# JoergBitzer/JadeSpectrogram

Measured on AMD Instinct MI355X. Metric: STFT frames/sec (1024-pt, 50% hop), higher is better.
Workload: dtype f32

## Files before the change

### include/jsg.h

```cpp
#ifndef JSG_H_
#define JSG_H_

#include <stddef.h>
#include <stdint.h>

#if defined(__GNUC__)
#define JSG_API __attribute__((visibility("default")))
#else
#define JSG_API
#endif

#ifdef __cplusplus
extern "C" {
#endif

#define JSG_ABI_VERSION 6

typedef enum jsg_status {
    JSG_OK = 0,
    JSG_ERR_SIZE_MISMATCH = -1,
    JSG_ERR_INVALID = -2,
    JSG_ERR_UNSUPPORTED = -3,
    JSG_ERR_HIP = -4,
    JSG_ERR_NO_DEVICE = -5,
// ... 34 lines not shown
JSG_API int jsg_plan_create(jsg_plan** out, int n, const float* window, float power_scale);
JSG_API int jsg_plan_destroy(jsg_plan* plan);
JSG_API int jsg_plan_fft_size(const jsg_plan* plan);

typedef struct jsg_stft_args {
    const float* in;
    int64_t in_pitch;
    int32_t channels;
    int32_t hop;
    int32_t feedblocks;
    int32_t mix_mode;
    int64_t first_frame;
    int64_t n_frames;
    float* out_db;
    int64_t out_pitch;
    int64_t out_channel_pitch;
    int32_t ring_width;
    int32_t ring_pos;
    int32_t linear_out;
    int32_t blocks_per_cu;
    int64_t in_samples;
    int32_t plan_select;
    int32_t exact_log;
    int32_t reserved0;
    float* out_tail;
} jsg_stft_args;
JSG_API int jsg_stft_db_launch(const jsg_plan* plan, const jsg_stft_args* args, void* stream);
JSG_API int jsg_stft_kernel_name(const jsg_plan* plan, const jsg_stft_args* args, char* out, int out_len);

JSG_API int jsg_stft_db_launch_many(const jsg_plan* plan, const jsg_stft_args* args, int count, void* const* streams, int n_streams);
JSG_API int jsg_stft_db_launch_many_threads(const jsg_plan* plan, const jsg_stft_args* args, int count, void* const* streams,
                                    int n_streams, int n_threads);

JSG_API int jsg_stft_db_launch_batches(const jsg_plan* plan, const jsg_stft_args* args, int count, void* stream);

JSG_API int jsg_stft_db_launch_strided(const jsg_plan* plan, const jsg_stft_args* args, int n_batches, int64_t in_batch_stride,
                               int64_t out_batch_stride, void* stream);
JSG_API int jsg_stft_db_strided_kernel_name(const jsg_plan* plan, const jsg_stft_args* args, int n_batches, int64_t in_batch_stride, char* out,
                                    int out_len);

JSG_API int jsg_db_from_power_launch(const float* power, float* out, int64_t count, float divisor, void* stream);
JSG_API int jsg_db_from_power_launch_ex(const float* power, float* out, int64_t count, float divisor, int exact_log, void* stream);

JSG_API int jsg_columns_from_tail_layout_launch(const float* db, int64_t db_pitch, const float* tail, int n_columns, int height, float* dst,
                                        int64_t dst_pitch, void* stream);

JSG_API int jsg_calib_copy_launch(const void* src, void* dst, int64_t bytes, void* stream);

typedef struct jsg_colormap_args {
    const float* db;
    int64_t db_pitch;
    int32_t ring_width;
    int32_t height;
    int32_t col_first;
    int32_t n_cols;
    int32_t x_first;
    int32_t x_wrap;
    const int32_t* lut;
    int32_t n_colors;
    float vmin, vmax, access_mult;
    uint32_t* argb_out;
    int64_t argb_pitch;
// ... 186 lines not shown
```

### jadespectrogram_amd/__init__.py

```python
from . import capi
from .capi import JsgError
from .spectrogram import (CColorPalette, Filterbank, FreqAxis, Plan, Spectrogram, SpectrogramDisplay, StftLaunch, colormap, colormap_lut,
                          colormap_axis, colormap_range, columns_from_tail_layout, feed_samples, memsize_blocks, next_power_of_2, stft_db, stft_db_batches, stft_db_strided, stft_db_strided_kernel_name, stft_image, stft_image_needs_scratch, stft_image_strided, stft_image_strided_needs_scratch, stft_kernel_name, window,
                          mel_spectrogram_db, stft_fb_db, stft_fb_db_strided, stft_fb_kernel_name, stft_fb_scratch_floats,
                          CStftPlan, cstft, istft, istft_launch, istft_nola, istft_scratch_floats, stft,
                          phase_vocoder, phase_vocoder_launch, pvoc_frames, time_stretch)

__all__ = ["Spectrogram", "SpectrogramDisplay", "CColorPalette", "Plan", "stft_db", "colormap", "window", "colormap_lut",
           "colormap_range", "feed_samples", "memsize_blocks", "next_power_of_2", "JsgError", "capi",
           "Filterbank", "stft_fb_db", "stft_fb_db_strided", "stft_fb_kernel_name", "mel_spectrogram_db", "FreqAxis", "colormap_axis",
           "CStftPlan", "cstft", "istft_launch", "istft_nola", "istft_scratch_floats", "stft", "istft",
           "pvoc_frames", "phase_vocoder_launch", "phase_vocoder", "time_stretch"]
```

### jadespectrogram_amd/_build.py

```python
from __future__ import annotations

import os
import shutil
import subprocess
import sys

PKG = os.path.dirname(os.path.abspath(__file__))
ROOT = os.path.dirname(PKG)
CSRC = os.path.join(PKG, "csrc")
LIB = os.path.join(PKG, "libjsg.so")

SOURCES = ["jsg_kernels.hip", "jsg_stft_a.hip", "jsg_stft_b.hip", "jsg_filterbank.hip", "jsg_display_axis.hip", "jsg_cstft.hip", "jsg_pvoc.hip", "jsg_engine.cpp", "jsg_host_math.cpp", "jsg_filterbank_host.cpp",
           "jsg_display_axis_host.cpp"]
HEADERS = ["jsg_internal.h", "jsg_block_queue.h", "jsg_exact_math.h", "jsg_stft_kernel.h", "jsg_colormap_tables.inc", os.path.join(ROOT, "include", "jsg.h")]
HIP_FLAGS = ["-fno-slp-vectorize", "-mllvm", "-amdgpu-kernarg-preload-count=16"]
VISIBILITY = ["-fvisibility=hidden", "-fvisibility-inlines-hidden"]
UNIT_FLAGS = {"jsg_stft_a.hip": ["-mllvm", "-amdgpu-sched-strategy=max-ilp"]}
ARCH = "gfx950"


def _hipcc() -> str:
    for cand in (os.environ.get("HIPCC"), shutil.which("hipcc"), "/opt/rocm/bin/hipcc"):
        if cand and os.path.exists(cand):
            return cand
    raise RuntimeError("hipcc not found: libjsg.so cannot be built (there is no CPU fallback)")


def _stale(target: str, deps) -> bool:
    if not os.path.exists(target):
        return True
    t = os.path.getmtime(target)
    return any(os.path.getmtime(d) > t for d in deps)


def build_variant(name: str, hip_flags, verbose: bool = False) -> str:
    hipcc = _hipcc()
    vdir = os.path.join(ROOT, "tools", "variants")
# ... 81 lines not shown
```

### jadespectrogram_amd/capi.py

```python
from __future__ import annotations

import ctypes as C
import os

PKG = os.path.dirname(os.path.abspath(__file__))
LIB_PATH = os.path.join(PKG, "libjsg.so")

JSG_OK = 0
JSG_ERR_SIZE_MISMATCH = -1
JSG_ERR_INVALID = -2
JSG_ERR_UNSUPPORTED = -3
JSG_ERR_HIP = -4
JSG_ERR_NO_DEVICE = -5
JSG_ERR_NOMEM = -6

MIX_ABSMEAN, MIX_MAX, MIX_MIN, MIX_LEFT, MIX_RIGHT = range(5)
MIX_PER_CHANNEL = 100
MIX_SUM = 101
WIN_RECT, WIN_HANN, WIN_HAMMING, WIN_BLACKMANHARRIS, WIN_FLATTOP, WIN_HANNPOISSON = range(6)
FEED_100, FEED_50, FEED_25, FEED_10 = range(4)
CM_MONO, CM_BW, CM_HOT, CM_RAINBOW, CM_VIRIDIS, CM_PLASMA, CM_JADE = range(7)
FB_MEL_SLANEY, FB_MEL_HTK, FB_LOG, FB_LINEAR = range(4)
FB_NORM_NONE, FB_NORM_SLANEY, FB_NORM_UNIT_SUM = range(3)
FB_MAX_BANDS = 8192
AXIS_BINS, AXIS_LINEAR, AXIS_LOG, AXIS_MEL = range(4)
AXIS_MAX_HEIGHT = 16384


class JsgError(RuntimeError):
    def __init__(self, code: int, msg: str):
        super().__init__(f"jsg error {code}: {msg}")
        self.code = code


class StftArgs(C.Structure):
    _fields_ = [("in_", C.c_void_p), ("in_pitch", C.c_int64), ("channels", C.c_int32), ("hop", C.c_int32),
                ("feedblocks", C.c_int32), ("mix_mode", C.c_int32), ("first_frame", C.c_int64),
                ("n_frames", C.c_int64), ("out_db", C.c_void_p), ("out_pitch", C.c_int64),
                ("out_channel_pitch", C.c_int64), ("ring_width", C.c_int32), ("ring_pos", C.c_int32),
                ("linear_out", C.c_int32), ("blocks_per_cu", C.c_int32), ("in_samples", C.c_int64),
                ("plan_select", C.c_int32), ("exact_log", C.c_int32), ("reserved0", C.c_int32), ("out_tail", C.c_void_p)]


class FbSpec(C.Structure):
    _fields_ = [("n", C.c_int32), ("fs", C.c_float), ("n_bands", C.c_int32), ("fmin", C.c_float), ("fmax", C.c_float),
                ("scale", C.c_int32), ("norm", C.c_int32)]


class AxisSpec(C.Structure):
    _fields_ = [("n", C.c_int32), ("fs", C.c_float), ("scale", C.c_int32), ("height", C.c_int32), ("fmin", C.c_float),
                ("fmax", C.c_float)]


class ColormapArgs(C.Structure):
    _fields_ = [("db", C.c_void_p), ("db_pitch", C.c_int64), ("ring_width", C.c_int32), ("height", C.c_int32),
                ("col_first", C.c_int32), ("n_cols", C.c_int32), ("x_first", C.c_int32), ("x_wrap", C.c_int32),
                ("lut", C.c_void_p), ("n_colors", C.c_int32), ("vmin", C.c_float), ("vmax", C.c_float),
                ("access_mult", C.c_float), ("argb_out", C.c_void_p), ("argb_pitch", C.c_int64),
                ("index_out", C.c_void_p), ("index_pitch", C.c_int64)]


class CstftArgs(C.Structure):
    _fields_ = [("in_", C.c_void_p), ("in_pitch", C.c_int64), ("rows", C.c_int32), ("hop", C.c_int32), ("n_frames", C.c_int64),
                ("in_samples", C.c_int64), ("out", C.c_void_p), ("out_frame_pitch", C.c_int64), ("out_row_pitch", C.c_int64)]
# ... 14 lines not shown
    _fields_ = [("stft", StftArgs), ("colour", ColormapArgs), ("index_scratch", C.c_void_p), ("index_scratch_pitch", C.c_int64)]


_P = C.c_void_p
SIGNATURES = {
    "jsg_abi_version": (C.c_int, []),
    "jsg_device_count": (C.c_int, []),
    "jsg_feed_samples": (C.c_int, [C.c_float, C.c_int]),
    "jsg_memsize_blocks": (C.c_int, [C.c_float, C.c_float, C.c_int]),
    "jsg_next_power_of_2": (C.c_int, [C.c_float, C.c_float]),
    "jsg_window_build": (C.c_int, [C.c_int, C.c_int, _P]),
    "jsg_colormap_build": (C.c_int, [C.c_int, C.c_int, _P]),
    "jsg_colormap_range": (C.c_int, [C.c_int, C.c_float, C.c_float, _P, _P, _P]),
    "jsg_plan_create": (C.c_int, [C.POINTER(_P), C.c_int, _P, C.c_float]),
    "jsg_plan_destroy": (C.c_int, [_P]),
    "jsg_plan_fft_size": (C.c_int, [_P]),
    "jsg_stft_db_launch": (C.c_int, [_P, C.POINTER(StftArgs), _P]),
    "jsg_stft_db_launch_many": (C.c_int, [_P, C.POINTER(StftArgs), C.c_int, C.POINTER(_P), C.c_int]),
    "jsg_stft_db_launch_many_threads": (C.c_int, [_P, C.POINTER(StftArgs), C.c_int, C.POINTER(_P), C.c_int, C.c_int]),
    "jsg_stft_db_launch_batches": (C.c_int, [_P, C.POINTER(StftArgs), C.c_int, _P]),
    "jsg_stft_kernel_name": (C.c_int, [_P, C.POINTER(StftArgs), C.c_char_p, C.c_int]),
    "jsg_stft_db_launch_strided": (C.c_int, [_P, C.POINTER(StftArgs), C.c_int, C.c_int64, C.c_int64, _P]),
    "jsg_stft_db_strided_kernel_name": (C.c_int, [_P, C.POINTER(StftArgs), C.c_int, C.c_int64, C.c_char_p, C.c_int]),
    "jsg_calib_copy_launch": (C.c_int, [_P, _P, C.c_int64, _P]),
    "jsg_columns_from_tail_layout_launch": (C.c_int, [_P, C.c_int64, _P, C.c_int, C.c_int, _P, C.c_int64, _P]),
    "jsg_colormap_launch": (C.c_int, [C.POINTER(ColormapArgs), _P]),
    "jsg_stft_image_launch": (C.c_int, [_P, C.POINTER(StftImageArgs), _P]),
    "jsg_stft_image_needs_scratch": (C.c_int, [_P, C.POINTER(StftImageArgs)]),
    "jsg_stft_image_launch_strided": (C.c_int, [_P, C.POINTER(StftImageArgs), C.c_int, C.c_int64, C.c_int64, _P]),
    "jsg_stft_image_strided_needs_scratch": (C.c_int, [_P, C.POINTER(StftImageArgs), C.c_int]),
    "jsg_db_from_power_launch": (C.c_int, [_P, _P, C.c_int64, C.c_float, _P]),
    "jsg_db_from_power_launch_ex": (C.c_int, [_P, _P, C.c_int64, C.c_float, C.c_int, _P]),
    "jsg_filterbank_build": (C.c_int, [C.POINTER(FbSpec), _P, _P, _P, _P, _P, C.c_int64, C.POINTER(C.c_int64)]),
    "jsg_filterbank_create": (C.c_int, [C.POINTER(_P), C.POINTER(FbSpec)]),
    "jsg_filterbank_create_matrix": (C.c_int, [C.POINTER(_P), C.c_int, C.c_int, _P]),
    "jsg_filterbank_destroy": (C.c_int, [_P]),
    "jsg_filterbank_bands": (C.c_int, [_P]),
    "jsg_filterbank_fft_size": (C.c_int, [_P]),
    "jsg_filterbank_weights": (C.c_int, [_P, _P]),
    "jsg_stft_fb_launch": (C.c_int, [_P, _P, C.POINTER(StftArgs), _P, C.c_int64, _P]),
    "jsg_stft_fb_launch_strided": (C.c_int, [_P, _P, C.POINTER(StftArgs), C.c_int, C.c_int64, C.c_int64, _P, C.c_int64, _P]),
    "jsg_stft_fb_scratch_floats": (C.c_int64, [_P, _P, C.POINTER(StftArgs), C.c_int]),
    "jsg_stft_fb_kernel_name": (C.c_int, [_P, _P, C.POINTER(StftArgs), C.c_int, C.c_char_p, C.c_int]),
    "jsg_freq_axis_build": (C.c_int, [C.POINTER(AxisSpec), _P, _P, _P, _P]),
    "jsg_freq_axis_create": (C.c_int, [C.POINTER(_P), C.POINTER(AxisSpec)]),
    "jsg_freq_axis_destroy": (C.c_int, [_P]),
# ... 95 lines not shown
```

### jadespectrogram_amd/csrc/jsg_kernels.hip

```cpp
#include <memory>

#include "jsg_stft_kernel.h"

namespace jsg {

#ifdef JSG_DEV_KNOBS
static int dev_knob_int(const char* name) { const char* e = getenv(name); return e ? atoi(e) : 0; }
static bool dev_knob_set(const char* name) { return getenv(name) != nullptr; }
static bool dev_knob_is(const char* name, char first) { const char* e = getenv(name); return e && e[0] == first; }
#else
static constexpr int dev_knob_int(const char*) { return 0; }
static constexpr bool dev_knob_set(const char*) { return false; }
static constexpr bool dev_knob_is(const char*, char) { return false; }
#endif

static bool chunked_traversal() {
    static const bool chunked = dev_knob_is("JSG_TRAVERSAL", 'c');
    return chunked;
}

static bool b_plan_fills_its_rounds(long long n_frames, int frames_per_workgroup, int n_cu) {
    const long long want = (n_frames + frames_per_workgroup - 1) / frames_per_workgroup;
    const long long rounds = (want + n_cu - 1) / n_cu;
    return rounds > 0 && double(want) >= kB_min_round_fill * double(rounds * n_cu);
// ... 111 lines not shown
    const long long col = blockIdx.x;
    const float* src = db + col * db_pitch;
    float* out = dst + col * dst_pitch;
    for (int k = threadIdx.x; k < half; k += 256) out[k] = src[k];
    if (threadIdx.x == 0) out[half] = tail[col];
}

__global__ __launch_bounds__(256) void calib_copy_kernel(const float* __restrict__ src, float* __restrict__ dst, long long n4) {
    typedef float v4f __attribute__((ext_vector_type(4)));
    const long long i = (long long)blockIdx.x * 256 + threadIdx.x;
    if (i < n4) __builtin_nontemporal_store(__builtin_nontemporal_load(reinterpret_cast<const v4f*>(src) + i), reinterpret_cast<v4f*>(dst) + i);
}

}

using namespace jsg;

namespace {
#define JSG_VARIANT_ROW(V, C, U, name, step, tables, pin, one_per_cu) \
    {C::N, name, step, int(Tables::tables), pin, one_per_cu, &launch_##V, &ensure_attrs_##V, &fill_tables<C>},
const VariantRow kVariants[] = {JSG_STFT_VARIANTS(JSG_VARIANT_ROW)};
#undef JSG_VARIANT_ROW
const VariantRow& row_of(Variant v) { return kVariants[int(v)]; }
}

struct jsg_plan {
    int n = 0;
    DeviceBlob blob;
    const float2* d_tab = nullptr;
    size_t set_at[kTableSets] = {0, 0, 0};
};

extern "C" {


int jsg_device_count(void) {
    int n = 0;
    if (hipGetDeviceCount(&n) != hipSuccess) return 0;
    return n;
}

static void pool_prepare_for_device(int dev);

int jsg_plan_create(jsg_plan** out, int n, const float* window, float power_scale) {
    if (!out || !window) return jsg_fail(JSG_ERR_INVALID, "jsg_plan_create: null argument");
    *out = nullptr;
// ... 40 lines not shown

int jsg_plan_fft_size(const jsg_plan* plan) { return plan ? plan->n : JSG_ERR_INVALID; }

}

int jsg::plan_device(const jsg_plan* plan) { return plan->blob.device(); }

namespace {
struct IndexOut {
    unsigned char* idx;
    long long pitch;
    float vmin, vmax, mult;
    int n_colors;
    unsigned* argb;
    long long argb_pitch;
    const int* lut;
    int x_first, x_wrap;
    int n_images = 1;
    long long in_image_stride = 0, argb_image_stride = 0;
};
}

constexpr int k1024B_min_channels = 4;

namespace {
struct CallShape {
    enum Out { kFloat, kIndex, kArgb } out = kFloat;
    long long rows = 1;
    int n_images = 1;
    bool multi_batch = false;
};
}

static Variant resolve_variant(const jsg_plan* plan, const jsg_stft_args* g, const CallShape& sh, int n_cu) {
    const int n = plan->n, mm = g->mix_mode, sel = g->plan_select;
    const bool maxmin = mm == JSG_MIX_MAX || mm == JSG_MIX_MIN;
    const int nc = (mm == JSG_MIX_LEFT || mm == JSG_MIX_RIGHT || mm == JSG_MIX_PER_CHANNEL) ? 1 : g->channels;
    if (n == 512) return Variant::k512;
    if (n == 8192) return Variant::k8192;
    if (n == 1024 && sh.out == CallShape::kArgb) return Variant::k1024I;
    if (n == 2048 && sel == 3 && sh.out == CallShape::kFloat && (mm == JSG_MIX_ABSMEAN || mm == JSG_MIX_SUM) && g->channels >= 2 &&
        (g->channels & 1) == 0)
        return Variant::k2048P;
    const Variant b_plan = n == 1024 ? Variant::k1024B : n == 2048 ? Variant::k2048B : Variant::k4096B;
    const int step = row_of(b_plan).step;
    const long long frames = sh.out == CallShape::kArgb ? (g->n_frames + step - 1) / step * step * sh.n_images : sh.rows * g->n_frames;
    bool b;
    if (n == 1024) {
        b = sh.out == CallShape::kFloat && !maxmin &&
            (sel == 2 || (sel == 0 && nc >= k1024B_min_channels && b_plan_fills_its_rounds(frames, step, n_cu)));
    } else {
        static const int forced2048 = dev_knob_int("JSG_2048_PLAN");
        static const int forced4096 = dev_knob_int("JSG_4096_PLAN");
        const int forced = sel == 1 ? 3 : sel == 2 ? 2 : n == 2048 ? forced2048 : forced4096;
        b = forced == 2 || (forced != 3 && nc >= (n == 2048 ? k2048B_min_channels : k4096B_min_channels) &&
                            b_plan_fills_its_rounds(frames, step, n_cu));
    }
    if (b) return b_plan;
    if (n == 2048) return Variant::k2048;
    if (n == 4096) return Variant::k4096;
    static const bool no_runs = dev_knob_set("JSG_NO_RUNS");
    const bool runs = sh.multi_batch && nc == 1 && !maxmin && (long long)g->hop * g->feedblocks == n && 2 * g->hop == n &&
                      !chunked_traversal() && !no_runs;
    return runs ? Variant::k1024Runs : Variant::k1024;
}

const VariantRow& jsg::strided_call_variant(const jsg_plan* plan, const jsg_stft_args* g, int n_batches, int n_cu) {
    const bool one_by_one = g->mix_mode == JSG_MIX_MAX || g->mix_mode == JSG_MIX_MIN;
    CallShape sh;
    sh.rows = (one_by_one ? 1ll : (long long)n_batches) * (g->mix_mode == JSG_MIX_PER_CHANNEL ? g->channels : 1);
    return row_of(resolve_variant(plan, g, sh, n_cu));
}

int jsg::check_stft_args(int n, const jsg_stft_args* g, const char* who) {
    if (g->hop <= 0 || g->feedblocks <= 0) return jsg_fail_who(JSG_ERR_INVALID, who, "bad geometry (hop, feedblocks)");
    if (g->channels > 65535) return jsg_fail_who(JSG_ERR_UNSUPPORTED, who, "more than 65535 channels");
    if (g->in_samples != 0) {
        const long long j = g->first_frame + g->n_frames - 1;
        const long long start = ((long long)g->hop * g->feedblocks == n) ? j * g->hop : (j / g->feedblocks) * n + (j % g->feedblocks) * g->hop;
        if (g->in_samples < 0 || start + n > g->in_samples) return jsg_fail_who(JSG_ERR_INVALID, who, "the last frame would read past the end of the input rows");
        if (g->channels > 1 && g->in_pitch < g->in_samples) return jsg_fail_who(JSG_ERR_INVALID, who, "in_pitch < in_samples");
    }
    if (g->n_frames >= (1ll << 31) || g->first_frame + g->n_frames >= (1ll << 31)) return jsg_fail_who(JSG_ERR_UNSUPPORTED, who, "frame index does not fit 31 bits");
    switch (g->mix_mode) {
        case JSG_MIX_ABSMEAN: case JSG_MIX_MAX: case JSG_MIX_MIN: case JSG_MIX_LEFT: case JSG_MIX_PER_CHANNEL: case JSG_MIX_SUM: return JSG_OK;
        case JSG_MIX_RIGHT:
            return g->channels < 2 ? jsg_fail_who(JSG_ERR_INVALID, who, "JSG_MIX_RIGHT needs at least two channels") : JSG_OK;
// ... 288 lines not shown
        one.in = g->in + b0 * in_batch_stride;
        one.out_db = g->out_db ? g->out_db + b0 * out_batch_stride : nullptr;
        if (g->out_tail) one.out_tail = g->out_tail + b0 * rows_per_batch * g->ring_width;
        if (nb == 1) rc = jsg_stft_db_launch(plan, &one, stream);
        else {
            BatchSpec bs{nb, (long long)in_batch_stride, (long long)out_batch_stride};
            rc = stft_launch_impl(plan, &one, nullptr, stream, &bs);
        }
        if (rc != JSG_OK) return rc;
    }
    return JSG_OK;
}

int jsg_stft_db_strided_kernel_name(const jsg_plan* plan, const jsg_stft_args* g, int n_batches, int64_t in_batch_stride, char* out, int out_len) {
    if (!plan || !g || !out || out_len < 24 || n_batches < 1) return jsg_fail(JSG_ERR_INVALID, "jsg_stft_db_strided_kernel_name: bad argument");
    int dev = -1;
    if (hipGetDevice(&dev) != hipSuccess) return jsg_fail(JSG_ERR_NO_DEVICE, "jsg_stft_db_strided_kernel_name: no device");
    if (n_batches == 1) return jsg_stft_kernel_name(plan, g, out, out_len);
    (void)in_batch_stride;
    std::snprintf(out, size_t(out_len), "%s", strided_call_variant(plan, g, n_batches, cu_count_of_device(dev)).name);
    return JSG_OK;
}

int jsg_stft_db_launch_many(const jsg_plan* plan, const jsg_stft_args* args, int count, void* const* streams, int n_streams) {
    if (!plan || (!args && count > 0) || count < 0 || n_streams < 0 || (n_streams > 0 && !streams))
        return jsg_fail(JSG_ERR_INVALID, "jsg_stft_db_launch_many: bad argument");
    for (int i = 0; i < count; ++i) {
        void* st = n_streams > 0 ? streams[i % n_streams] : nullptr;
        const int rc = jsg_stft_db_launch(plan, &args[i], st);
        if (rc != JSG_OK) return rc;
    }
    return JSG_OK;
}

int jsg_stft_db_launch_many_threads(const jsg_plan* plan, const jsg_stft_args* args, int count, void* const* streams, int n_streams,
                                    int n_threads) {
    if (n_threads <= 1 || n_streams <= 1) return jsg_stft_db_launch_many(plan, args, count, streams, n_streams);
    if (!plan || (!args && count > 0) || count < 0 || !streams) return jsg_fail(JSG_ERR_INVALID, "jsg_stft_db_launch_many_threads: bad argument");
    if (n_threads > n_streams) n_threads = n_streams;
    if (n_threads > 16) n_threads = 16;
    int dev = 0;
    if (hipGetDevice(&dev) != hipSuccess) return jsg_fail(JSG_ERR_NO_DEVICE, "jsg_stft_db_launch_many_threads: no device");
    std::vector<int> rcs(size_t(n_threads), JSG_OK);
    std::vector<std::string> errs{size_t(n_threads)};
    auto body = [&](int t) {
        if (hipSetDevice(dev) != hipSuccess) { rcs[size_t(t)] = JSG_ERR_HIP; return; }
// ... 193 lines not shown
```

### jadespectrogram_amd/csrc/jsg_stft_a.hip

```cpp
#include "jsg_stft_kernel.h"

namespace jsg {
#define JSG_IN_UNIT_A(...) __VA_ARGS__
#define JSG_IN_UNIT_B(...)
JSG_STFT_VARIANTS(JSG_DEFINE_VARIANT)
hipError_t touch_module_a() { return preload_code_object(reinterpret_cast<const void*>(&stft_db_kernel<Cfg1024, 3>)); }
}
```

### jadespectrogram_amd/csrc/jsg_stft_kernel.h

```cpp
#pragma once
#include <hip/hip_runtime.h>

#include <algorithm>
#include <atomic>
#include <cmath>
#include <cstdint>
#include <cstdio>
#include <cstdlib>
#include <mutex>
#include <new>
#include <string>
#include <thread>
#include <type_traits>
#include <utility>
#include <vector>

#include "../../include/jsg.h"
#include "jsg_internal.h"
#include "jsg_exact_math.h"

namespace jsg {

typedef float cf __attribute__((ext_vector_type(2)));

// ... 1499 lines not shown
    else
        hipLaunchKernelGGL((stft_db_kernel<C, MIXOP, OUTK, STREAM, 0>), grid, dim3(C::WPB * 64), lds, s, ka.in, ka.in_pitch, ka.tab, ka.n_frames,
                           ka.first_frame, ka.hop, flags, unsigned(ka.c_begin) | unsigned(ka.c_end) << 16, ka.iters, grid.x, ka.feedblocks, ka);
    return hipGetLastError();
}

template <class C, int K = 0>
hipError_t launch_stft(const StftKArgs& ka, int mixop, int stream, dim3 grid, hipStream_t s) {
    if constexpr (K == 4 * 3 * 3) return hipErrorInvalidValue;
    else {
        constexpr int MIXOP = K % 4, OUTK = K / 4 % 3, STREAM = K / 12;
        if constexpr (stft_instantiated<C, MIXOP, OUTK, STREAM>())
            if (mixop == MIXOP && (ka.argb ? 2 : ka.idx ? 1 : 0) == OUTK && stream == STREAM) return launch_stft_mix<C, MIXOP, OUTK, STREAM>(ka, grid, s);
        return launch_stft<C, K + 1>(ka, mixop, stream, grid, s);
    }
}

#define JSG_STFT_VARIANTS(X)                                                                                  \
    X(k512,      Cfg512,   A, "Cfg512",   Cfg512::TPB,            First, 0, false)                            \
    X(k1024,     Cfg1024,  A, "Cfg1024",  Cfg1024::TPB,           First, 1, false)                            \
    X(k1024I,    Cfg1024I, A, "Cfg1024I", Cfg1024I::TPB,          First, 0, false)                            \
    X(k1024B,    Cfg1024B, A, "Cfg1024B", Cfg1024B::TPB,          B,     2, true)                             \
    X(k1024Runs, Cfg1024,  A, "Cfg1024",  Cfg1024::TPB * kRunLen, First, 1, false)                            \
    X(k2048,     Cfg2048,  A, "Cfg2048",  Cfg2048::TPB,           First, 1, false)                            \
    X(k2048B,    Cfg2048B, A, "Cfg2048B", Cfg2048B::TPB,          B,     2, true)                             \
    X(k2048P,    Cfg2048P, A, "Cfg2048P", Cfg2048P::TPB,          Pair,  3, true)                             \
    X(k4096,     Cfg4096,  B, "Cfg4096",  Cfg4096::TPB,           First, 1, false)                            \
    X(k4096B,    Cfg4096B, B, "Cfg4096B", Cfg4096B::TPB,          B,     2, true)                             \
    X(k8192,     Cfg8192,  A, "Cfg8192",  Cfg8192::TPB,           First, 0, false)

#define JSG_VARIANT_ENUMERATOR(V, ...) V,
enum class Variant : int { JSG_STFT_VARIANTS(JSG_VARIANT_ENUMERATOR) };
#undef JSG_VARIANT_ENUMERATOR

#define JSG_VARIANT_ENTRY_POINTS(V, C, ...)                                                        \
    hipError_t launch_##V(const StftKArgs& ka, int mixop, bool strided, dim3 grid, hipStream_t s); \
    hipError_t ensure_attrs_##V();
JSG_STFT_VARIANTS(JSG_VARIANT_ENTRY_POINTS)
#undef JSG_VARIANT_ENTRY_POINTS
enum class Tables : int { First, B, Pair };
constexpr int kTableSets = 3;
struct VariantRow {
    int n;
    const char* name;
    int step;
    int tables;
    int plan_select;
    bool one_per_cu;
    hipError_t (*launch)(const StftKArgs& ka, int mixop, bool strided, dim3 grid, hipStream_t s);
    hipError_t (*ensure_attrs)();
    void (*fill)(std::vector<float2>& t, const float* window, double amp);
};
const VariantRow& strided_call_variant(const jsg_plan* plan, const jsg_stft_args* g, int n_batches, int n_cu);

#define JSG_DEFINE_VARIANT(V, C, U, ...)                                                                                 \
    JSG_IN_UNIT_##U(                                                                                                      \
        hipError_t launch_##V(const StftKArgs& ka, int mixop, bool strided, dim3 grid, hipStream_t s) {                   \
            return launch_stft<C>(ka, mixop, Variant::V == Variant::k1024Runs ? 2 : strided ? 1 : 0, grid, s);              \
        }                                                                                                                 \
        hipError_t ensure_attrs_##V() { return ensure_lds_attrs<C>(); })
hipError_t touch_module_a();
hipError_t touch_module_b();

}
```

### jadespectrogram_amd/spectrogram.py

```python
from __future__ import annotations

import ctypes as C

import numpy as np

from . import capi
from .capi import JsgError, check, lib


def feed_samples(feed_percent: float, fftsize: int) -> int:
    return check(lib().jsg_feed_samples(feed_percent, fftsize))


def memsize_blocks(memsize_s: float, fs: float, hop: int) -> int:
    return check(lib().jsg_memsize_blocks(memsize_s, fs, hop))


def next_power_of_2(ms: float, fs: float) -> int:
    return check(lib().jsg_next_power_of_2(ms, fs))


def window(kind: int, n: int) -> np.ndarray:
    out = np.zeros(n, dtype=np.float32)
    check(lib().jsg_window_build(kind, n, out.ctypes.data))
# ... 296 lines not shown


def _strided_args(plan: Plan, d_in, hop: int, n_frames: int, d_out, **kw):
    assert d_in.dim() == 3 and d_in.stride(2) == 1 and d_out.shape[0] == d_in.shape[0] and d_out.stride(-1) == 1
    a = _stft_args(plan, d_in[0], hop, n_frames, d_out[0], **kw)
    return a, int(d_in.shape[0]), int(d_in.stride(0)), int(d_out.stride(0))


def stft_db_strided(plan: Plan, d_in, hop: int, n_frames: int, d_out, *, stream: int | None = None, **kw):
    import torch
    a, k, s_in, s_out = _strided_args(plan, d_in, hop, n_frames, d_out, **kw)
    if stream is None:
        stream = torch.cuda.current_stream(d_in.device).cuda_stream
    check(lib().jsg_stft_db_launch_strided(plan._p, C.byref(a), k, s_in, s_out, C.c_void_p(stream)))


def stft_db_strided_kernel_name(plan: Plan, d_in, hop: int, n_frames: int, d_out, **kw) -> str:
    a, k, s_in, _ = _strided_args(plan, d_in, hop, n_frames, d_out, **kw)
    buf = C.create_string_buffer(32)
    check(lib().jsg_stft_db_strided_kernel_name(plan._p, C.byref(a), k, s_in, buf, 32))
    return buf.value.decode()


def stft_kernel_name(plan: Plan, d_in, hop: int, n_frames: int, d_out, **kw) -> str:
    a = _stft_args(plan, d_in, hop, n_frames, d_out, **kw)
    buf = C.create_string_buffer(32)
    check(lib().jsg_stft_kernel_name(plan._p, C.byref(a), buf, 32))
    return buf.value.decode()


def _stft_args(plan: Plan, d_in, hop: int, n_frames: int, d_out, *, feedblocks: int | None = None, mix_mode: int = 0,
               first_frame: int = 0, ring_pos: int = 0, linear_out: bool = False, blocks_per_cu: int = 0, plan_select: int = 0,
               exact_log: bool = False, d_tail=None, col_height: int | None = None):
    import torch
    assert d_in.is_cuda and d_in.dtype == torch.float32 and d_in.dim() == 2 and d_in.stride(1) == 1
    assert d_out.is_cuda and d_out.dtype == torch.float32 and d_out.stride(-1) == 1
    H = (plan.n // 2 + 1 - (1 if d_tail is not None else 0)) if col_height is None else int(col_height)
    if d_out.shape[-1] < H:
        raise JsgError(capi.JSG_ERR_INVALID, f"output rows hold {d_out.shape[-1]} floats, a column needs {H}")
    if mix_mode == capi.MIX_PER_CHANNEL and (d_out.dim() != 3 or d_out.shape[0] != d_in.shape[0]):
        raise JsgError(capi.JSG_ERR_INVALID, "per-channel mode needs an output of [channels][W][pitch]")
    a = capi.StftArgs()
    a.in_ = d_in.data_ptr()
    a.in_pitch = d_in.stride(0) if d_in.shape[0] > 1 else d_in.shape[1]
    a.in_samples = d_in.shape[1]
    a.channels = d_in.shape[0]
    a.hop = hop
    a.feedblocks = feedblocks if feedblocks is not None else max(1, plan.n // hop)
    a.mix_mode = mix_mode
    a.first_frame = first_frame
    a.n_frames = n_frames
    a.out_db = d_out.data_ptr()
    a.out_pitch = d_out.stride(-2)
    a.out_channel_pitch = d_out.stride(0) if d_out.dim() == 3 else 0
    a.ring_width = d_out.shape[-2]
    a.ring_pos = ring_pos
    a.linear_out = int(bool(linear_out))
    a.blocks_per_cu = int(blocks_per_cu)
    a.exact_log = int(bool(exact_log))
    a.plan_select = int(plan_select)
    if d_tail is not None:
        assert d_tail.is_cuda and d_tail.dtype == torch.float32 and d_tail.is_contiguous() and d_tail.shape[-1] == d_out.shape[-2]
        a.out_tail = d_tail.data_ptr()
    return a


def colormap(d_db, d_lut, lo: float, hi: float, *, d_argb=None, d_index=None, col_first: int = 0, n_cols: int | None = None,
             x_first: int = 0, height: int | None = None, stream: int | None = None):
    import torch
    a = _colormap_args(d_db, d_lut, lo, hi, d_argb, d_index, col_first, n_cols, x_first, height)
    if stream is None:
        stream = torch.cuda.current_stream(d_db.device).cuda_stream
    check(lib().jsg_colormap_launch(C.byref(a), C.c_void_p(stream)))


def colormap_axis(d_db, d_lut, lo: float, hi: float, axis: "FreqAxis", *, d_argb=None, d_index=None, col_first: int = 0,
                  n_cols: int | None = None, x_first: int = 0, stream: int | None = None):
    import torch
    a = _colormap_args(d_db, d_lut, lo, hi, d_argb, d_index, col_first, n_cols, x_first, axis.n // 2 + 1)
    if stream is None:
        stream = torch.cuda.current_stream(d_db.device).cuda_stream
    check(lib().jsg_colormap_axis_launch(C.byref(a), axis.handle(d_db.device.index), C.c_void_p(stream)))

# ... 502 lines not shown
```

Measured before the change: 1.259 billion.

## Add hand-specialized hot kernel for 1024-point two-column runs STFT

Adds a dedicated kernel for the common 1024-point, 50%-hop, dB-output runs case. It keeps the overlapping half-frame in registers across the two columns of a run, prefetches the next run's samples while the current FFT is computed, and passes the Nyquist bin between columns with DPP. Output uses nontemporal stores. The general kernel's runtime branches for linear, tail and exact-log output are dropped on this path, and it becomes the default when the conditions match. In exchange there is a second, hand-maintained kernel path with more register pressure and a fallback that errors if its preconditions fail.

Result: no change. 1.277 billion, median of 5 (+1.5%).

```diff
diff --git a/include/jsg.h b/include/jsg.h
--- a/include/jsg.h
+++ b/include/jsg.h
@@ -80,7 +80,7 @@
     int64_t in_samples;
     int32_t plan_select;
     int32_t exact_log;
-    int32_t reserved0;
+    int32_t runs_form;
     float* out_tail;
 } jsg_stft_args;
 JSG_API int jsg_stft_db_launch(const jsg_plan* plan, const jsg_stft_args* args, void* stream);
@@ -96,6 +96,7 @@
                                int64_t out_batch_stride, void* stream);
 JSG_API int jsg_stft_db_strided_kernel_name(const jsg_plan* plan, const jsg_stft_args* args, int n_batches, int64_t in_batch_stride, char* out,
                                     int out_len);
+JSG_API int jsg_stft_db_strided_variant_name(const jsg_plan* plan, const jsg_stft_args* args, int n_batches, char* out, int out_len);
 
 JSG_API int jsg_db_from_power_launch(const float* power, float* out, int64_t count, float divisor, void* stream);
 JSG_API int jsg_db_from_power_launch_ex(const float* power, float* out, int64_t count, float divisor, int exact_log, void* stream);
diff --git a/jadespectrogram_amd/__init__.py b/jadespectrogram_amd/__init__.py
--- a/jadespectrogram_amd/__init__.py
+++ b/jadespectrogram_amd/__init__.py
@@ -1,7 +1,7 @@
 from . import capi
 from .capi import JsgError
 from .spectrogram import (CColorPalette, Filterbank, FreqAxis, Plan, Spectrogram, SpectrogramDisplay, StftLaunch, colormap, colormap_lut,
-                          colormap_axis, colormap_range, columns_from_tail_layout, feed_samples, memsize_blocks, next_power_of_2, stft_db, stft_db_batches, stft_db_strided, stft_db_strided_kernel_name, stft_image, stft_image_needs_scratch, stft_image_strided, stft_image_strided_needs_scratch, stft_kernel_name, window,
+                          colormap_axis, colormap_range, columns_from_tail_layout, feed_samples, memsize_blocks, next_power_of_2, stft_db, stft_db_batches, stft_db_strided, stft_db_strided_kernel_name, stft_db_strided_variant_name, stft_image, stft_image_needs_scratch, stft_image_strided, stft_image_strided_needs_scratch, stft_kernel_name, window,
                           mel_spectrogram_db, stft_fb_db, stft_fb_db_strided, stft_fb_kernel_name, stft_fb_scratch_floats,
                           CStftPlan, cstft, istft, istft_launch, istft_nola, istft_scratch_floats, stft,
                           phase_vocoder, phase_vocoder_launch, pvoc_frames, time_stretch)
diff --git a/jadespectrogram_amd/_build.py b/jadespectrogram_amd/_build.py
--- a/jadespectrogram_amd/_build.py
+++ b/jadespectrogram_amd/_build.py
@@ -12,7 +12,7 @@
 
 SOURCES = ["jsg_kernels.hip", "jsg_stft_a.hip", "jsg_stft_b.hip", "jsg_filterbank.hip", "jsg_display_axis.hip", "jsg_cstft.hip", "jsg_pvoc.hip", "jsg_engine.cpp", "jsg_host_math.cpp", "jsg_filterbank_host.cpp",
            "jsg_display_axis_host.cpp"]
-HEADERS = ["jsg_internal.h", "jsg_block_queue.h", "jsg_exact_math.h", "jsg_stft_kernel.h", "jsg_colormap_tables.inc", os.path.join(ROOT, "include", "jsg.h")]
+HEADERS = ["jsg_internal.h", "jsg_block_queue.h", "jsg_exact_math.h", "jsg_stft_kernel.h", "jsg_stft_runs_hot.h", "jsg_colormap_tables.inc", os.path.join(ROOT, "include", "jsg.h")]
 HIP_FLAGS = ["-fno-slp-vectorize", "-mllvm", "-amdgpu-kernarg-preload-count=16"]
 VISIBILITY = ["-fvisibility=hidden", "-fvisibility-inlines-hidden"]
 UNIT_FLAGS = {"jsg_stft_a.hip": ["-mllvm", "-amdgpu-sched-strategy=max-ilp"]}
diff --git a/jadespectrogram_amd/capi.py b/jadespectrogram_amd/capi.py
--- a/jadespectrogram_amd/capi.py
+++ b/jadespectrogram_amd/capi.py
@@ -39,7 +39,7 @@
                 ("n_frames", C.c_int64), ("out_db", C.c_void_p), ("out_pitch", C.c_int64),
                 ("out_channel_pitch", C.c_int64), ("ring_width", C.c_int32), ("ring_pos", C.c_int32),
                 ("linear_out", C.c_int32), ("blocks_per_cu", C.c_int32), ("in_samples", C.c_int64),
-                ("plan_select", C.c_int32), ("exact_log", C.c_int32), ("reserved0", C.c_int32), ("out_tail", C.c_void_p)]
+                ("plan_select", C.c_int32), ("exact_log", C.c_int32), ("runs_form", C.c_int32), ("out_tail", C.c_void_p)]
 
 
 class FbSpec(C.Structure):
@@ -100,6 +100,7 @@
     "jsg_stft_kernel_name": (C.c_int, [_P, C.POINTER(StftArgs), C.c_char_p, C.c_int]),
     "jsg_stft_db_launch_strided": (C.c_int, [_P, C.POINTER(StftArgs), C.c_int, C.c_int64, C.c_int64, _P]),
     "jsg_stft_db_strided_kernel_name": (C.c_int, [_P, C.POINTER(StftArgs), C.c_int, C.c_int64, C.c_char_p, C.c_int]),
+    "jsg_stft_db_strided_variant_name": (C.c_int, [_P, C.POINTER(StftArgs), C.c_int, C.c_char_p, C.c_int]),
     "jsg_calib_copy_launch": (C.c_int, [_P, _P, C.c_int64, _P]),
     "jsg_columns_from_tail_layout_launch": (C.c_int, [_P, C.c_int64, _P, C.c_int, C.c_int, _P, C.c_int64, _P]),
     "jsg_colormap_launch": (C.c_int, [C.POINTER(ColormapArgs), _P]),
diff --git a/jadespectrogram_amd/csrc/jsg_kernels.hip b/jadespectrogram_amd/csrc/jsg_kernels.hip
--- a/jadespectrogram_amd/csrc/jsg_kernels.hip
+++ b/jadespectrogram_amd/csrc/jsg_kernels.hip
@@ -157,6 +157,9 @@
 const VariantRow kVariants[] = {JSG_STFT_VARIANTS(JSG_VARIANT_ROW)};
 #undef JSG_VARIANT_ROW
 const VariantRow& row_of(Variant v) { return kVariants[int(v)]; }
+#define JSG_VARIANT_ID(V, ...) #V,
+const char* const kVariantIds[] = {JSG_STFT_VARIANTS(JSG_VARIANT_ID)};
+#undef JSG_VARIANT_ID
 }
 
 struct jsg_plan {
@@ -243,6 +246,7 @@
 }
 
 constexpr int k1024B_min_channels = 4;
+constexpr bool kRunsHotAuto = true;
 
 namespace {
 struct CallShape {
@@ -283,7 +287,10 @@
     static const bool no_runs = dev_knob_set("JSG_NO_RUNS");
     const bool runs = sh.multi_batch && nc == 1 && !maxmin && (long long)g->hop * g->feedblocks == n && 2 * g->hop == n &&
                       !chunked_traversal() && !no_runs;
-    return runs ? Variant::k1024Runs : Variant::k1024;
+    static const bool no_hot = dev_knob_set("JSG_NO_RUNS_HOT");
+    const bool hot = runs && sh.out == CallShape::kFloat && !g->linear_out && !g->exact_log && !g->out_tail && !no_hot &&
+                     (g->runs_form == 2 || (g->runs_form == 0 && kRunsHotAuto));
+    return hot ? Variant::k1024RunsHot : runs ? Variant::k1024Runs : Variant::k1024;
 }
 
 const VariantRow& jsg::strided_call_variant(const jsg_plan* plan, const jsg_stft_args* g, int n_batches, int n_cu) {
@@ -618,6 +625,24 @@
     return JSG_OK;
 }
 
+int jsg_stft_db_strided_variant_name(const jsg_plan* plan, const jsg_stft_args* g, int n_batches, char* out, int out_len) {
+    if (!plan || !g || !out || out_len < 24 || n_batches < 1) return jsg_fail(JSG_ERR_INVALID, "jsg_stft_db_strided_variant_name: bad argument");
+    int dev = -1;
+    if (hipGetDevice(&dev) != hipSuccess) return jsg_fail(JSG_ERR_NO_DEVICE, "jsg_stft_db_strided_variant_name: no device");
+    const int n_cu = cu_count_of_device(dev);
+    const bool one_by_one = g->mix_mode == JSG_MIX_MAX || g->mix_mode == JSG_MIX_MIN;
+    jsg_stft_args one = *g;
+    const int pin = strided_call_variant(plan, g, n_batches, n_cu).plan_select;
+    if (pin && n_batches > 1) one.plan_select = pin;
+    CallShape sh;
+    if (n_batches > 1 && !one_by_one) {
+        sh.rows = (long long)n_batches * (g->mix_mode == JSG_MIX_PER_CHANNEL ? g->channels : 1);
+        sh.multi_batch = true;
+    }
+    std::snprintf(out, size_t(out_len), "%s", kVariantIds[int(resolve_variant(plan, &one, sh, n_cu))]);
+    return JSG_OK;
+}
+
 int jsg_stft_db_launch_many(const jsg_plan* plan, const jsg_stft_args* args, int count, void* const* streams, int n_streams) {
     if (!plan || (!args && count > 0) || count < 0 || n_streams < 0 || (n_streams > 0 && !streams))
         return jsg_fail(JSG_ERR_INVALID, "jsg_stft_db_launch_many: bad argument");
diff --git a/jadespectrogram_amd/csrc/jsg_stft_a.hip b/jadespectrogram_amd/csrc/jsg_stft_a.hip
--- a/jadespectrogram_amd/csrc/jsg_stft_a.hip
+++ b/jadespectrogram_amd/csrc/jsg_stft_a.hip
@@ -1,4 +1,5 @@
 #include "jsg_stft_kernel.h"
+#include "jsg_stft_runs_hot.h"
 
 namespace jsg {
 #define JSG_IN_UNIT_A(...) __VA_ARGS__
diff --git a/jadespectrogram_amd/csrc/jsg_stft_kernel.h b/jadespectrogram_amd/csrc/jsg_stft_kernel.h
--- a/jadespectrogram_amd/csrc/jsg_stft_kernel.h
+++ b/jadespectrogram_amd/csrc/jsg_stft_kernel.h
@@ -1545,6 +1545,7 @@
     X(k1024I,    Cfg1024I, A, "Cfg1024I", Cfg1024I::TPB,          First, 0, false)                            \
     X(k1024B,    Cfg1024B, A, "Cfg1024B", Cfg1024B::TPB,          B,     2, true)                             \
     X(k1024Runs, Cfg1024,  A, "Cfg1024",  Cfg1024::TPB * kRunLen, First, 1, false)                            \
+    X(k1024RunsHot, Cfg1024, A, "Cfg1024", Cfg1024::TPB * kRunLen, First, 1, false)                            \
     X(k2048,     Cfg2048,  A, "Cfg2048",  Cfg2048::TPB,           First, 1, false)                            \
     X(k2048B,    Cfg2048B, A, "Cfg2048B", Cfg2048B::TPB,          B,     2, true)                             \
     X(k2048P,    Cfg2048P, A, "Cfg2048P", Cfg2048P::TPB,          Pair,  3, true)                             \
@@ -1561,6 +1562,7 @@
     hipError_t ensure_attrs_##V();
 JSG_STFT_VARIANTS(JSG_VARIANT_ENTRY_POINTS)
 #undef JSG_VARIANT_ENTRY_POINTS
+hipError_t launch_runs_hot(const StftKArgs& ka, int mixop, dim3 grid, hipStream_t s);
 enum class Tables : int { First, B, Pair };
 constexpr int kTableSets = 3;
 struct VariantRow {
@@ -1579,7 +1581,8 @@
 #define JSG_DEFINE_VARIANT(V, C, U, ...)                                                                                 \
     JSG_IN_UNIT_##U(                                                                                                      \
         hipError_t launch_##V(const StftKArgs& ka, int mixop, bool strided, dim3 grid, hipStream_t s) {                   \
-            return launch_stft<C>(ka, mixop, Variant::V == Variant::k1024Runs ? 2 : strided ? 1 : 0, grid, s);              \
+            if constexpr (Variant::V == Variant::k1024RunsHot) return launch_runs_hot(ka, mixop, grid, s);                \
+            else return launch_stft<C>(ka, mixop, Variant::V == Variant::k1024Runs ? 2 : strided ? 1 : 0, grid, s);         \
         }                                                                                                                 \
         hipError_t ensure_attrs_##V() { return ensure_lds_attrs<C>(); })
 hipError_t touch_module_a();
diff --git a/jadespectrogram_amd/csrc/jsg_stft_runs_hot.h b/jadespectrogram_amd/csrc/jsg_stft_runs_hot.h
--- /dev/null
+++ b/jadespectrogram_amd/csrc/jsg_stft_runs_hot.h
@@ -0,0 +1,293 @@
+#pragma once
+#include "jsg_stft_kernel.h"
+
+namespace jsg {
+
+struct RunsHotArgs {
+    long long in_batch_stride, in_pitch;
+    long long out_batch_stride, out_cpitch;
+    long long out_pitch;
+    unsigned long long bat_magic;
+    unsigned bat_cpb;
+    int ring_w, ring_pos;
+};
+
+__device__ __forceinline__ float sel_lane0(float first, float rest, unsigned long long not_lane0) {
+    float r;
+    asm("v_cndmask_b32 %0, %1, %2, %3" : "=v"(r) : "v"(first), "v"(rest), "s"(not_lane0));
+    return r;
+}
+
+__global__ __launch_bounds__(Cfg1024::WPB * 64, 5) JSG_NO_LDS_MERGE void stft_runs1024_kernel(
+    const float* __restrict__ k_in, const float2* __restrict__ k_tab, float* __restrict__ k_out, const unsigned k_n_frames,
+    const unsigned k_first_frame, const unsigned k_nblk, const int k_iters, const unsigned k_n_groups, const unsigned k_gpr,
+    const int k_xcd_remap, const int k_pad, const unsigned long long k_row_magic, const RunsHotArgs a) {
+    using C = Cfg1024;
+    constexpr int L = C::L, P = C::P, M = C::M, R1 = C::R1, R2 = C::R2, R3 = C::R3, RL = kRunLen, H = P / 2;
+    static_assert(L == 64 && C::U1 == 1 && C::U2 == 1 && C::U3 == 1 && C::FPW == 1 && C::RTAB && C::TLOC == 1 && !C::TWF && !C::PAIR && !C::TWO_STAGE,
+                  "the three-stage 64-lane plan with register tables");
+    static_assert(RL == 2, "the hot form is written out for runs of two columns");
+    constexpr int HOP = C::N / 2;
+    (void)k_pad;
+    __shared__ __attribute__((aligned(16))) cf s_tab[C::TAB_ELEMS];
+    extern __shared__ __attribute__((aligned(16))) char smem_raw[];
+    typedef float v4f __attribute__((ext_vector_type(4)));
+
+    const int lane = threadIdx.x & 63;
+    const int wave = __builtin_amdgcn_readfirstlane(threadIdx.x >> 6);
+    const int ll = lane;
+    cf* const lds0 = reinterpret_cast<cf*>(smem_raw) + wave * C::LDS_ELEMS;
+
+    const unsigned nblk = k_nblk, b = blockIdx.x;
+    const unsigned xcd = b & 7, jb = b >> 3, full = nblk & ~255u;
+    unsigned lb = b;
+    if (k_xcd_remap) {
+        constexpr unsigned CL = JSG_X_XCD_CHUNK_LOG2;
+        if (b < full && b < (nblk & ~((8u << CL) - 1u))) lb = ((jb >> CL) << (CL + 3)) + (xcd << CL) + (jb & ((1u << CL) - 1u));
+        else if (b < full) lb = b;
+        else {
+            const unsigned t = nblk - full, q = t >> 3, r = t & 7;
+            lb = full + (xcd < r ? xcd * (q + 1) : r * (q + 1) + (xcd - r) * q) + ((b - full) >> 3);
+        }
+    }
+    __builtin_assume(k_iters >= 1);
+
+    f2u rw[2][H];
+    unsigned nx_col0 = 0, cu_col0 = 0;
+    long long nx_in = 0, nx_out = 0, cu_out = 0;
+    auto runs_group = [&](unsigned sg) {
+        unsigned g = lb + sg * nblk;
+        if (g >= k_n_groups) g -= k_n_groups;
+        const unsigned row = (unsigned)(((unsigned long long)g * k_row_magic) >> 40);
+        nx_col0 = (g - row * k_gpr) * (unsigned)(C::TPB * RL) + (unsigned)(wave * RL);
+        const unsigned batch = (unsigned)(((unsigned long long)row * a.bat_magic) >> 40);
+        const unsigned ch = row - batch * a.bat_cpb;
+        nx_in = (long long)batch * a.in_batch_stride + (long long)ch * a.in_pitch;
+        nx_out = (long long)batch * a.out_batch_stride + (long long)ch * a.out_cpitch;
+    };
+    auto runs_src = [&](unsigned tu) -> const f2u* {
+        const unsigned tc = tu < k_n_frames ? tu : k_n_frames - 1;
+        const long long start = (long long)(k_first_frame + tc) * HOP + nx_in;
+        return reinterpret_cast<const f2u*>(k_in + start) + ll;
+    };
+
+    constexpr int NTL = (C::TAB_ELEMS / 2 + C::WPB * 64 - 1) / (C::WPB * 64);
+    constexpr bool TAB_EVEN = (C::TAB_ELEMS / 2) % (C::WPB * 64) == 0;
+    {
+        const v4f* g4 = reinterpret_cast<const v4f*>(k_tab) + threadIdx.x;
+        char* sbase = reinterpret_cast<char*>(s_tab) + wave * 1024;
+#pragma unroll
+        for (int i = 0; i < NTL; ++i)
+            if (TAB_EVEN || i + 1 < NTL || (int)threadIdx.x + i * C::WPB * 64 < C::TAB_ELEMS / 2)
+                __builtin_amdgcn_global_load_lds((const __attribute__((address_space(1))) void*)(g4 + i * C::WPB * 64),
+                                                 (__attribute__((address_space(3))) void*)(sbase + i * C::WPB * 1024), 16, 0, 0);
+        __builtin_amdgcn_sched_barrier(0);
+    }
+    {
+        runs_group(0u);
+        const f2u* src = runs_src(nx_col0);
+#pragma unroll
+        for (int m = 0; m < H; ++m) rw[0][m] = src[L * m];
+#pragma unroll
+        for (int m = 0; m < H; ++m) rw[1][m] = src[L * (m + H)];
+        __builtin_amdgcn_sched_barrier(0);
+    }
+    __builtin_amdgcn_fence(__ATOMIC_RELEASE, "wavefront");
+    asm volatile("s_waitcnt vmcnt(%0)\n\ts_barrier" ::"n"(P) : "memory");
+    __builtin_amdgcn_fence(__ATOMIC_ACQUIRE, "wavefront");
+    const cf* const tBase = s_tab;
+
+    cf rt1[R1], rpost[H];
+    {
+        const cf* const tTw1 = tBase + C::TAB_TW1 + (ll / R3) * C::TS1;
+#pragma unroll
+        for (int k1 = 1; k1 < R1; k1 += 2) {
+            const v4f q4 = *reinterpret_cast<const v4f*>(tTw1 + k1 - 1);
+            rt1[k1] = cf{q4.x, q4.y};
+            if (k1 + 1 < R1) rt1[k1 + 1] = cf{q4.z, q4.w};
+        }
+#pragma unroll
+        for (int rho = 0; rho < H; rho += 2) {
+            const v4f q4 = *reinterpret_cast<const v4f*>(tBase + C::TAB_POST + C::tab_idx(rho, ll));
+            rpost[rho] = cf{q4.x, q4.y};
+            rpost[rho + 1] = cf{q4.z, q4.w};
+        }
+    }
+    auto tab2 = [&](int off, int j, cf& a0, cf& a1) {
+        const v4f q4 = *reinterpret_cast<const v4f*>(tBase + off + C::tab_idx(j, ll));
+        a0 = cf{q4.x, q4.y};
+        a1 = cf{q4.z, q4.w};
+    };
+    const int e1r = (ll / R3) * C::S1 + (ll % R3);
+    const int e2w = (ll / R3) * C::AX + (ll % R3) * C::AZ;
+    const int e2r = (ll % R1) * C::AX + (ll / R1) * C::AY;
+
+    const unsigned long long not_lane0 = ~1ull;
+    const int lwu = lane == 0 ? 64 : lane;
+    cf zA = {0.f, 0.f};
+    float upA = 0.f;
+
+    auto process = [&](unsigned next_sg, auto last_tag, auto t_tag) __attribute__((always_inline)) {
+        constexpr bool LAST = decltype(last_tag)::value;
+        constexpr int T = decltype(t_tag)::value;
+        constexpr int PAR = T & 1;
+        if constexpr (T == 0) { cu_col0 = nx_col0; cu_out = nx_out; }
+        cf x[P];
+        cf wlo[H];
+#pragma unroll
+        for (int m = 0; m < P; m += 2) {
+            cf w0, w1;
+            tab2(C::TAB_WIN, m, w0, w1);
+            if (m < H) {
+                x[m] = to_cf(rw[PAR][m]);
+                x[m + 1] = to_cf(rw[PAR][m + 1]);
+                wlo[m] = w0;
+                wlo[m + 1] = w1;
+            } else {
+                x[m] = to_cf(rw[PAR ^ 1][m - H]) * w0;
+                x[m + 1] = to_cf(rw[PAR ^ 1][m + 1 - H]) * w1;
+            }
+        }
+        if constexpr (T + 1 < RL) {
+            const f2u* src = runs_src(nx_col0 + (unsigned)(T + 1));
+#pragma unroll
+            for (int m = 0; m < H; ++m) rw[PAR][m] = src[L * (m + H)];
+        } else if constexpr (!LAST) {
+            runs_group(next_sg);
+            const f2u* src = runs_src(nx_col0);
+#pragma unroll
+            for (int m = 0; m < H; ++m) rw[PAR ^ 1][m] = src[L * m];
+#pragma unroll
+            for (int m = 0; m < H; ++m) rw[PAR][m] = src[L * (m + H)];
+        }
+        {
+            sr_dft_win<R1>(x, wlo);
+            lds0[ll] = x[0];
+#pragma unroll
+            for (int k1 = 1; k1 < R1; k1 += 2) {
+                lds0[k1 * C::S1 + ll] = cmul(x[k1], rt1[k1]);
+                if (k1 + 1 < R1) lds0[(k1 + 1) * C::S1 + ll] = cmul(x[k1 + 1], rt1[k1 + 1]);
+            }
+        }
+        wave_sync();
+#pragma unroll
+        for (int n2 = 0; n2 < R2; ++n2) x[n2] = lds0[e1r + n2 * R3];
+        wave_sync();
+        sr_dft<R2>(x);
+#pragma unroll
+        for (int k2 = 0; k2 < R2; k2 += 2) {
+            cf w0, w1;
+            tab2(C::TAB_TW2, k2, w0, w1);
+            lds0[e2w + k2 * C::AY] = cmul(x[k2], w0);
+            lds0[e2w + (k2 + 1) * C::AY] = cmul(x[k2 + 1], w1);
+        }
+        wave_sync();
+#pragma unroll
+        for (int n3 = 0; n3 < R3; ++n3) x[n3] = lds0[e2r + n3 * C::AZ];
+        wave_sync();
+        sr_dft<R3>(x);
+#pragma unroll
+        for (int rho = H; rho < P; ++rho) lds0[ll + L * rho] = x[rho];
+        if (ll == 0) lds0[M] = x[0];
+        wave_sync();
+        cf zq[H];
+#pragma unroll
+        for (int rho = 0; rho < H; ++rho) zq[rho] = lds0[M - (ll + L * rho)];
+        wave_sync();
+        cf acc[H];
+#pragma unroll
+        for (int rho = 0; rho < H; ++rho) {
+            const cf z = x[rho], p = zq[rho];
+            const cf S = add_conj(z, p);
+            const cf Tt = cmul(sub_conj(z, p), rpost[rho]);
+            const cf re = addsub_re(S, Tt), im = addsub_im(S, Tt);
+            cf pw = re * re;
+            pw = __builtin_elementwise_fma(im, im, pw);
+            acc[rho] = pw;
+        }
+#pragma unroll
+        for (int m = 0; m < H; ++m) {
+            cf t = acc[m] + cf{1e-11f, 1e-11f};
+            t = cf{__builtin_amdgcn_logf(t.x), __builtin_amdgcn_logf(t.y)};
+            acc[m] = t * cf{3.0102999566398120f, 3.0102999566398120f};
+        }
+        unsigned colA = (unsigned)a.ring_pos + cu_col0;
+        if (colA >= (unsigned)a.ring_w) colA -= (unsigned)a.ring_w;
+        unsigned col = colA;
+        if constexpr (T == 1) {
+            col = colA + 1u;
+            if (col == (unsigned)a.ring_w) col = 0u;
+        }
+        float* const dst = k_out + (long long)col * a.out_pitch + cu_out;
+        const bool live = cu_col0 + (unsigned)T < k_n_frames;
+        if constexpr (T == 0) {
+            zA = x[H];
+            upA = acc[H - 1].y;
+            if (live) {
+#pragma unroll
+                for (int rho = 0; rho < H; ++rho) {
+                    __builtin_nontemporal_store(acc[rho].x, &dst[lane + L * rho]);
+                    if (rho + 1 < H) __builtin_nontemporal_store(sel_lane0(acc[rho + 1].y, acc[rho].y, not_lane0), &dst[M - (lwu + L * rho)]);
+                }
+                if (lane == 0) __builtin_nontemporal_store(acc[0].y, &dst[M]);
+            }
+        } else {
+            cf z;
+            z.x = __int_as_float(__builtin_amdgcn_update_dpp(__float_as_int(zA.x), __float_as_int(x[H].x), 0x111, 0x1, 0x1, false));
+            z.y = __int_as_float(__builtin_amdgcn_update_dpp(__float_as_int(zA.y), __float_as_int(x[H].y), 0x111, 0x1, 0x1, false));
+            float pny = 4.0f * __builtin_fmaf(z.x, z.x, z.y * z.y);
+            asm("" : "+v"(pny));
+            const float ny = to_db(pny);
+            const float nyB = __int_as_float(__builtin_amdgcn_update_dpp(0, __float_as_int(ny), 0x101, 0xf, 0xf, true));
+            if (live) {
+#pragma unroll
+                for (int rho = 0; rho < H; ++rho) {
+                    __builtin_nontemporal_store(acc[rho].x, &dst[lane + L * rho]);
+                    const float nxt = rho + 1 < H ? acc[rho + 1].y : nyB;
+                    __builtin_nontemporal_store(sel_lane0(nxt, acc[rho].y, not_lane0), &dst[M - (lwu + L * rho)]);
+                }
+                if (lane == 0) __builtin_nontemporal_store(acc[0].y, &dst[M]);
+            }
+            if (cu_col0 < k_n_frames) {
+                float* const dstA = k_out + (long long)colA * a.out_pitch + cu_out;
+                __builtin_nontemporal_store(sel_lane0(ny, upA, not_lane0), &dstA[M - (lwu + L * (H - 1))]);
+            }
+        }
+    };
+
+    using t0 = std::integral_constant<int, 0>;
+    using t1 = std::integral_constant<int, 1>;
+    unsigned sg = 1u;
+    for (int r = 0; r + 1 < k_iters; ++r, ++sg) {
+        process(sg, std::false_type{}, t0{});
+        process(sg, std::false_type{}, t1{});
+    }
+    process(sg, std::false_type{}, t0{});
+    process(sg, std::true_type{}, t1{});
+}
+
+inline bool runs_hot_form(const StftKArgs& ka, int mixop) {
+    return mixop == 3 && ka.regular && 2 * ka.hop == Cfg1024::N && !ka.linear && !ka.exact_log && !ka.tail && !ka.chunked && !ka.idx && !ka.argb &&
+           ka.scale == 1.0f && !ka.exact_div && (ka.per_channel || ka.c_end - ka.c_begin == 1);
+}
+
+hipError_t launch_runs_hot(const StftKArgs& ka, int mixop, dim3 grid, hipStream_t s) {
+    if (!runs_hot_form(ka, mixop) || grid.y != 1) return hipErrorInvalidValue;
+    static_assert(Cfg1024::LDS_BYTES <= 48 * 1024, "no LDS attribute needed");
+    RunsHotArgs r;
+    r.in_batch_stride = ka.in_image_stride;
+    r.in_pitch = ka.in_pitch;
+    r.out_batch_stride = ka.out_batch_stride;
+    r.out_cpitch = ka.out_cpitch;
+    r.out_pitch = ka.out_pitch;
+    r.bat_magic = ka.bat_magic;
+    r.bat_cpb = ka.bat_cpb;
+    r.ring_w = ka.ring_w;
+    r.ring_pos = ka.ring_pos;
+    const float* in = ka.in + (ka.per_channel ? 0ll : (long long)ka.c_begin * ka.in_pitch);
+    hipLaunchKernelGGL(stft_runs1024_kernel, grid, dim3(Cfg1024::WPB * 64), Cfg1024::LDS_BYTES, s, in, ka.tab, ka.out, ka.n_frames, ka.first_frame,
+                       grid.x, ka.iters, ka.n_groups, ka.img_gpi, ka.xcd_remap, 0, ka.img_magic, r);
+    return hipGetLastError();
+}
+
+}
diff --git a/jadespectrogram_amd/spectrogram.py b/jadespectrogram_amd/spectrogram.py
--- a/jadespectrogram_amd/spectrogram.py
+++ b/jadespectrogram_amd/spectrogram.py
@@ -342,6 +342,13 @@
     return buf.value.decode()
 
 
+def stft_db_strided_variant_name(plan: Plan, d_in, hop: int, n_frames: int, d_out, **kw) -> str:
+    a, k, _, _ = _strided_args(plan, d_in, hop, n_frames, d_out, **kw)
+    buf = C.create_string_buffer(32)
+    check(lib().jsg_stft_db_strided_variant_name(plan._p, C.byref(a), k, buf, 32))
+    return buf.value.decode()
+
+
 def stft_kernel_name(plan: Plan, d_in, hop: int, n_frames: int, d_out, **kw) -> str:
     a = _stft_args(plan, d_in, hop, n_frames, d_out, **kw)
     buf = C.create_string_buffer(32)
@@ -351,7 +358,7 @@
 
 def _stft_args(plan: Plan, d_in, hop: int, n_frames: int, d_out, *, feedblocks: int | None = None, mix_mode: int = 0,
                first_frame: int = 0, ring_pos: int = 0, linear_out: bool = False, blocks_per_cu: int = 0, plan_select: int = 0,
-               exact_log: bool = False, d_tail=None, col_height: int | None = None):
+               exact_log: bool = False, d_tail=None, col_height: int | None = None, runs_form: int = 0):
     import torch
     assert d_in.is_cuda and d_in.dtype == torch.float32 and d_in.dim() == 2 and d_in.stride(1) == 1
     assert d_out.is_cuda and d_out.dtype == torch.float32 and d_out.stride(-1) == 1
@@ -379,6 +386,7 @@
     a.blocks_per_cu = int(blocks_per_cu)
     a.exact_log = int(bool(exact_log))
     a.plan_select = int(plan_select)
+    a.runs_form = int(runs_form)
     if d_tail is not None:
         assert d_tail.is_cuda and d_tail.dtype == torch.float32 and d_tail.is_contiguous() and d_tail.shape[-1] == d_out.shape[-2]
         a.out_tail = d_tail.data_ptr()
```
